# Boese0601/MagicDance

Hardware: NVIDIA H100
Metric: denoise-steps/sec @512x512 50-step DDIM (higher is better)
Workload: dtype f16

## Files before the change

include/magicdance_b200.h:

```cpp
#ifndef MAGICDANCE_B200_H_
#define MAGICDANCE_B200_H_

#include <stdint.h>

#ifdef __cplusplus
extern "C" {
#endif

#define MDB_OK 0
#define MDB_ERR_INVALID (-1)
#define MDB_ERR_CUDA (-2)
#define MDB_ERR_UNSUPPORTED (-3)

#define MDB_ABI_VERSION 2

typedef void* mdb_stream_t;

int mdb_abi_version(void);
const char* mdb_last_error(void);
int mdb_device_check(void);
int64_t mdb_launch_count(void);
int64_t mdb_abi_struct_bytes(int32_t which);

#define MDB_TUNE_GEMM_PAIR_MIN_TILES 1
#define MDB_TUNE_ATTN40_2Q_MIN_CTAS 3
#define MDB_TUNE_GEMM_BN80_BELOW 4
int mdb_set_tuning(int32_t key, int32_t value);
int32_t mdb_get_tuning(int32_t key);

#define MDB_EPI_NONE 0
#define MDB_EPI_GEGLU 1

typedef struct mdb_gemm_desc {
  const void* a;
  int64_t lda;
  const void* a2;
  int64_t lda2;
  int32_t k1;
  int32_t conv;
  int32_t nb, h, w, c;
  const void* b;
  int64_t ldb;
  void* d;
  int64_t ldd;
  const float* bias;
  int64_t bias_batch_stride;
  int32_t rows_per_batch;
  int32_t epilogue;
  const void* residual;
  int64_t ldr;
  int32_t m, n, k;
  int32_t splits;
  float* splitk_ws;
  const float* ln_u;
  float ln_eps;
} mdb_gemm_desc;

int mdb_gemm_f16(const mdb_gemm_desc* desc, mdb_stream_t stream);

#define MDB_DTYPE_F16 0
#define MDB_DTYPE_F32 1

typedef struct mdb_gemm_bwd_desc {
  mdb_gemm_desc fwd;
  const void* dd; int64_t lddd;
  void* da; int64_t ldda; int32_t da_dtype; int32_t da_accumulate;
  void* da2; int64_t ldda2; int32_t da2_dtype; int32_t da2_accumulate;
  void* db; int64_t lddb; int32_t db_dtype; int32_t db_accumulate;
  float* dbias; int32_t dbias_accumulate;
  int32_t splits;
  float* ws;
} mdb_gemm_bwd_desc;

int mdb_gemm_bwd_f16(const mdb_gemm_bwd_desc* desc, mdb_stream_t stream);
int64_t mdb_gemm_bwd_ws_floats(const mdb_gemm_bwd_desc* desc);

typedef struct mdb_attn_desc {
  const void* q; int64_t ldq;
  const void* k0; int64_t ldk0; const void* vt0; int64_t ldvt0; int32_t n0; int32_t kv0_batches; int32_t ldv0_batch;
  const void* k1; int64_t ldk1; const void* vt1; int64_t ldvt1; int32_t n1; int32_t kv1_batches; int32_t ldv1_batch;
  void* out; int64_t ldo;
  int32_t batch, heads, d, nq;
  int32_t bank_batches;
  float scale;
} mdb_attn_desc;

int mdb_attention_f16(const mdb_attn_desc* desc, mdb_stream_t stream);

int mdb_attention_lse_f16(const mdb_attn_desc* desc, float* lse, mdb_stream_t stream);

typedef struct mdb_attn_bwd_desc {
  mdb_attn_desc fwd;
  const void* dout; int64_t lddout;
  const float* lse;
  void* dq; int64_t lddq;
  void* dk0; int64_t lddk0; void* dvt0; int64_t lddvt0;
  void* dk1; int64_t lddk1; void* dvt1; int64_t lddvt1;
  float* ws;
} mdb_attn_bwd_desc;

int mdb_attention_bwd_f16(const mdb_attn_bwd_desc* desc, mdb_stream_t stream);
int64_t mdb_attention_bwd_ws_floats(int32_t batch, int32_t heads, int32_t nq);

int mdb_groupnorm_f16(const void* x1, int32_t c1, const void* x2, int32_t c2, const float* gamma, const float* beta,
                      void* y, float* ws, int32_t batch, int32_t hw, float eps, int32_t silu, int32_t mode,
                      mdb_stream_t stream);
int64_t mdb_groupnorm_ws_floats(int32_t c, int32_t batch, int32_t hw);

int mdb_layernorm_f16(const void* x, const float* gamma, const float* beta, void* y, int64_t rows, int32_t c,
                      float eps, mdb_stream_t stream);

typedef struct mdb_groupnorm_bwd_desc {
  const void* x1; const void* x2; int32_t c1; int32_t c2;
  const float* gamma; const float* beta;
  const void* dy;
  int32_t batch; int32_t hw; float eps; int32_t silu;
  void* dx1; int32_t dx1_dtype; int32_t dx1_accumulate;
  void* dx2; int32_t dx2_dtype; int32_t dx2_accumulate;
  float* dgamma; float* dbeta; int32_t dgamma_accumulate; int32_t dbeta_accumulate;
  float* ws;
} mdb_groupnorm_bwd_desc;

int mdb_groupnorm_bwd_f16(const mdb_groupnorm_bwd_desc* desc, mdb_stream_t stream);
int64_t mdb_groupnorm_bwd_ws_floats(const mdb_groupnorm_bwd_desc* desc);

typedef struct mdb_layernorm_bwd_desc {
  const void* x; const float* gamma; const void* dy;
  int64_t rows; int32_t c; float eps;
  void* dx; int32_t dx_dtype; int32_t dx_accumulate;
  float* dgamma; float* dbeta; int32_t dgamma_accumulate; int32_t dbeta_accumulate;
  float* ws;
} mdb_layernorm_bwd_desc;

int mdb_layernorm_bwd_f16(const mdb_layernorm_bwd_desc* desc, mdb_stream_t stream);
int64_t mdb_layernorm_bwd_ws_floats(const mdb_layernorm_bwd_desc* desc);

int mdb_geglu_f16(const void* h, int64_t ldh, void* out, int64_t ldo, int64_t m, int32_t n, mdb_stream_t stream);
int mdb_geglu_bwd_f16(const void* h, int64_t ldh, const void* dout, int64_t lddout, void* dh, int64_t lddh, int64_t m,
                      int32_t n, mdb_stream_t stream);

int mdb_conv3x3_direct_f16(const void* x, const void* wt, const float* bias, const void* residual, void* y,
                           int32_t batch, int32_t h, int32_t w, int32_t cin, int32_t cout, int32_t stride,
                           int32_t silu, mdb_stream_t stream);

typedef struct mdb_conv3x3_bwd_desc {
  const void* x; const void* wt; const void* wt_t; const float* bias; const void* dy;
  int32_t batch; int32_t h; int32_t w; int32_t cin; int32_t cout; int32_t stride; int32_t silu;
  void* dx;
  float* dw; int32_t dw_accumulate;
  float* dbias; int32_t dbias_accumulate;
  float* ws;
} mdb_conv3x3_bwd_desc;

int mdb_conv3x3_direct_bwd_f16(const mdb_conv3x3_bwd_desc* desc, mdb_stream_t stream);
int64_t mdb_conv3x3_direct_bwd_ws_floats(const mdb_conv3x3_bwd_desc* desc);

int mdb_im2col3x3_f16(const void* x, void* col, int32_t batch, int32_t h, int32_t w, int32_t c, int32_t stride,
                      mdb_stream_t stream);

int mdb_im2col3x3_br_f16(const void* x, void* col, int32_t batch, int32_t h, int32_t w, int32_t c, int32_t stride,
                         mdb_stream_t stream);

int mdb_upsample2x_f16(const void* x, void* y, int32_t batch, int32_t h, int32_t w, int32_t c, mdb_stream_t stream);
int mdb_upsample2x_bwd_f16(const void* dy, void* dx, int32_t dx_dtype, int32_t accumulate, int32_t batch, int32_t h,
                           int32_t w, int32_t c, mdb_stream_t stream);

int mdb_add_f16(const void* a, const void* b, void* y, int64_t n_per_batch, int32_t batch, int32_t b_batches,
                mdb_stream_t stream);

int mdb_timestep_embedding_f32(const int64_t* t, int32_t t_count, float* out, int32_t batch, int32_t dim,
                               mdb_stream_t stream);

int mdb_skinny_linear_f32(const float* x, const void* w, const float* bias, float* out, int32_t rows, int32_t n,
                          int32_t k, int32_t silu_in, int32_t silu_out, mdb_stream_t stream);

typedef struct mdb_skinny_linear_bwd_desc {
  const float* x; const void* w; const float* dy;
  int32_t rows; int32_t n; int32_t k; int32_t silu_in;
  float* dx; int32_t dx_accumulate;
  float* dw; int32_t dw_accumulate;
  float* dbias; int32_t dbias_accumulate;
// ... 21 lines not shown
```

magicdance_b200/_lib.py:

```python
from __future__ import annotations

import ctypes as C
import os

from . import build as _build

c_void_p, c_int32, c_int64, c_float = C.c_void_p, C.c_int32, C.c_int64, C.c_float


class GemmDesc(C.Structure):
    _fields_ = [
        ("a", c_void_p), ("lda", c_int64), ("a2", c_void_p), ("lda2", c_int64),
        ("k1", c_int32), ("conv", c_int32), ("nb", c_int32), ("h", c_int32), ("w", c_int32), ("c", c_int32),
        ("b", c_void_p), ("ldb", c_int64), ("d", c_void_p), ("ldd", c_int64),
        ("bias", c_void_p), ("bias_batch_stride", c_int64), ("rows_per_batch", c_int32), ("epilogue", c_int32),
        ("residual", c_void_p), ("ldr", c_int64),
        ("m", c_int32), ("n", c_int32), ("k", c_int32), ("splits", c_int32), ("splitk_ws", c_void_p),
        ("ln_u", c_void_p), ("ln_eps", c_float),
    ]


class AttnDesc(C.Structure):
    _fields_ = [
        ("q", c_void_p), ("ldq", c_int64),
        ("k0", c_void_p), ("ldk0", c_int64), ("vt0", c_void_p), ("ldvt0", c_int64),
        ("n0", c_int32), ("kv0_batches", c_int32), ("ldv0_batch", c_int32),
        ("k1", c_void_p), ("ldk1", c_int64), ("vt1", c_void_p), ("ldvt1", c_int64),
        ("n1", c_int32), ("kv1_batches", c_int32), ("ldv1_batch", c_int32),
        ("out", c_void_p), ("ldo", c_int64),
        ("batch", c_int32), ("heads", c_int32), ("d", c_int32), ("nq", c_int32), ("bank_batches", c_int32),
        ("scale", c_float),
    ]


class AttnBwdDesc(C.Structure):
    _fields_ = [
        ("fwd", AttnDesc),
        ("dout", c_void_p), ("lddout", c_int64),
        ("lse", c_void_p),
        ("dq", c_void_p), ("lddq", c_int64),
        ("dk0", c_void_p), ("lddk0", c_int64), ("dvt0", c_void_p), ("lddvt0", c_int64),
        ("dk1", c_void_p), ("lddk1", c_int64), ("dvt1", c_void_p), ("lddvt1", c_int64),
        ("ws", c_void_p),
    ]


class GemmBwdDesc(C.Structure):
    _fields_ = [
        ("fwd", GemmDesc),
        ("dd", c_void_p), ("lddd", c_int64),
        ("da", c_void_p), ("ldda", c_int64), ("da_dtype", c_int32), ("da_accumulate", c_int32),
        ("da2", c_void_p), ("ldda2", c_int64), ("da2_dtype", c_int32), ("da2_accumulate", c_int32),
        ("db", c_void_p), ("lddb", c_int64), ("db_dtype", c_int32), ("db_accumulate", c_int32),
        ("dbias", c_void_p), ("dbias_accumulate", c_int32),
        ("splits", c_int32),
        ("ws", c_void_p),
    ]


class GroupNormBwdDesc(C.Structure):
    _fields_ = [
        ("x1", c_void_p), ("x2", c_void_p), ("c1", c_int32), ("c2", c_int32),
        ("gamma", c_void_p), ("beta", c_void_p),
        ("dy", c_void_p),
        ("batch", c_int32), ("hw", c_int32), ("eps", c_float), ("silu", c_int32),
        ("dx1", c_void_p), ("dx1_dtype", c_int32), ("dx1_accumulate", c_int32),
        ("dx2", c_void_p), ("dx2_dtype", c_int32), ("dx2_accumulate", c_int32),
        ("dgamma", c_void_p), ("dbeta", c_void_p), ("dgamma_accumulate", c_int32), ("dbeta_accumulate", c_int32),
        ("ws", c_void_p),
    ]


class LayerNormBwdDesc(C.Structure):
    _fields_ = [
        ("x", c_void_p), ("gamma", c_void_p), ("dy", c_void_p),
        ("rows", c_int64), ("c", c_int32), ("eps", c_float),
        ("dx", c_void_p), ("dx_dtype", c_int32), ("dx_accumulate", c_int32),
        ("dgamma", c_void_p), ("dbeta", c_void_p), ("dgamma_accumulate", c_int32), ("dbeta_accumulate", c_int32),
        ("ws", c_void_p),
    ]


class Conv3x3BwdDesc(C.Structure):
    _fields_ = [
        ("x", c_void_p), ("wt", c_void_p), ("wt_t", c_void_p), ("bias", c_void_p), ("dy", c_void_p),
        ("batch", c_int32), ("h", c_int32), ("w", c_int32), ("cin", c_int32), ("cout", c_int32), ("stride", c_int32),
        ("silu", c_int32),
        ("dx", c_void_p),
        ("dw", c_void_p), ("dw_accumulate", c_int32),
        ("dbias", c_void_p), ("dbias_accumulate", c_int32),
        ("ws", c_void_p),
    ]


class SkinnyBwdDesc(C.Structure):
    _fields_ = [
        ("x", c_void_p), ("w", c_void_p), ("dy", c_void_p),
        ("rows", c_int32), ("n", c_int32), ("k", c_int32), ("silu_in", c_int32),
        ("dx", c_void_p), ("dx_accumulate", c_int32),
        ("dw", c_void_p), ("dw_accumulate", c_int32),
        ("dbias", c_void_p), ("dbias_accumulate", c_int32),
        ("ws", c_void_p),
    ]


SIGNATURES = {
    "mdb_abi_version": (c_int32, []),
    "mdb_last_error": (C.c_char_p, []),
    "mdb_device_check": (c_int32, []),
    "mdb_launch_count": (c_int64, []),
    "mdb_abi_struct_bytes": (c_int64, [c_int32]),
    "mdb_set_tuning": (c_int32, [c_int32, c_int32]),
    "mdb_get_tuning": (c_int32, [c_int32]),
    "mdb_gemm_f16": (c_int32, [C.POINTER(GemmDesc), c_void_p]),
    "mdb_gemm_bwd_f16": (c_int32, [C.POINTER(GemmBwdDesc), c_void_p]),
    "mdb_gemm_bwd_ws_floats": (c_int64, [C.POINTER(GemmBwdDesc)]),
    "mdb_attention_f16": (c_int32, [C.POINTER(AttnDesc), c_void_p]),
    "mdb_attention_lse_f16": (c_int32, [C.POINTER(AttnDesc), c_void_p, c_void_p]),
    "mdb_attention_bwd_f16": (c_int32, [C.POINTER(AttnBwdDesc), c_void_p]),
    "mdb_attention_bwd_ws_floats": (c_int64, [c_int32, c_int32, c_int32]),
    "mdb_groupnorm_f16": (c_int32, [c_void_p, c_int32, c_void_p, c_int32, c_void_p, c_void_p, c_void_p, c_void_p,
                                    c_int32, c_int32, c_float, c_int32, c_int32, c_void_p]),
    "mdb_groupnorm_ws_floats": (c_int64, [c_int32, c_int32, c_int32]),
    "mdb_layernorm_f16": (c_int32, [c_void_p, c_void_p, c_void_p, c_void_p, c_int64, c_int32, c_float, c_void_p]),
    "mdb_groupnorm_bwd_f16": (c_int32, [C.POINTER(GroupNormBwdDesc), c_void_p]),
    "mdb_groupnorm_bwd_ws_floats": (c_int64, [C.POINTER(GroupNormBwdDesc)]),
    "mdb_layernorm_bwd_f16": (c_int32, [C.POINTER(LayerNormBwdDesc), c_void_p]),
    "mdb_layernorm_bwd_ws_floats": (c_int64, [C.POINTER(LayerNormBwdDesc)]),
    "mdb_geglu_f16": (c_int32, [c_void_p, c_int64, c_void_p, c_int64, c_int64, c_int32, c_void_p]),
    "mdb_geglu_bwd_f16": (c_int32, [c_void_p, c_int64, c_void_p, c_int64, c_void_p, c_int64, c_int64, c_int32,
                                    c_void_p]),
    "mdb_conv3x3_direct_f16": (c_int32, [c_void_p, c_void_p, c_void_p, c_void_p, c_void_p, c_int32, c_int32, c_int32,
                                         c_int32, c_int32, c_int32, c_int32, c_void_p]),
    "mdb_conv3x3_direct_bwd_f16": (c_int32, [C.POINTER(Conv3x3BwdDesc), c_void_p]),
    "mdb_conv3x3_direct_bwd_ws_floats": (c_int64, [C.POINTER(Conv3x3BwdDesc)]),
    "mdb_im2col3x3_f16": (c_int32, [c_void_p, c_void_p, c_int32, c_int32, c_int32, c_int32, c_int32, c_void_p]),
    "mdb_im2col3x3_br_f16": (c_int32, [c_void_p, c_void_p, c_int32, c_int32, c_int32, c_int32, c_int32, c_void_p]),
    "mdb_upsample2x_f16": (c_int32, [c_void_p, c_void_p, c_int32, c_int32, c_int32, c_int32, c_void_p]),
    "mdb_upsample2x_bwd_f16": (c_int32, [c_void_p, c_void_p, c_int32, c_int32, c_int32, c_int32, c_int32, c_int32,
                                         c_void_p]),
    "mdb_add_f16": (c_int32, [c_void_p, c_void_p, c_void_p, c_int64, c_int32, c_int32, c_void_p]),
    "mdb_timestep_embedding_f32": (c_int32, [c_void_p, c_int32, c_void_p, c_int32, c_int32, c_void_p]),
    "mdb_skinny_linear_f32": (c_int32, [c_void_p, c_void_p, c_void_p, c_void_p, c_int32, c_int32, c_int32, c_int32,
                                        c_int32, c_void_p]),
    "mdb_skinny_linear_bwd_f32": (c_int32, [C.POINTER(SkinnyBwdDesc), c_void_p]),
    "mdb_skinny_linear_bwd_ws_floats": (c_int64, [C.POINTER(SkinnyBwdDesc)]),
    "mdb_nchw_f32_to_nhwc_f16": (c_int32, [c_void_p, c_void_p, c_int32, c_int32, c_int32, c_int32, c_int32, c_void_p]),
    "mdb_nhwc_f16_to_nchw_f32": (c_int32, [c_void_p, c_void_p, c_int32, c_int32, c_int32, c_int32, c_void_p]),
    "mdb_softmax_rows_f16": (c_int32, [c_void_p, c_int64, c_int32, c_int32, c_float, c_void_p]),
    "mdb_cfg_ddim_update_f32": (c_int32, [c_void_p, c_void_p, c_void_p, c_void_p, c_void_p, c_void_p, c_int64,
                                          c_void_p, c_int32, c_void_p]),
}

_lib = None
ABI_VERSION = 2
TUNE_GEMM_PAIR_MIN_TILES, TUNE_ATTN40_2Q_MIN_CTAS, TUNE_GEMM_BN80_BELOW = 1, 3, 4


def library_path() -> str:
    return os.environ.get("MAGICDANCE_B200_LIB", _build.LIB_PATH)


def load():
    global _lib
    if _lib is not None:
        return _lib
    path = library_path()
    if not os.path.isfile(path):
        raise RuntimeError(
            f"magicdance_b200: kernel library {path} is missing — run `python -m magicdance_b200.build` "
            "(there is no CPU/PyTorch fallback for the hot path)")
    if path == _build.LIB_PATH and os.path.isdir(_build.CSRC) and not _build.is_fresh():
        raise RuntimeError(f"magicdance_b200: {path} was not built from the sources in {_build.CSRC} "
                           "(stamp mismatch) — run `python -m magicdance_b200.build`")
    lib = C.CDLL(path)
    for name, (res, args) in SIGNATURES.items():
        fn = getattr(lib, name)
        fn.restype = res
        fn.argtypes = args
    if lib.mdb_abi_version() != ABI_VERSION:
        raise RuntimeError(f"magicdance_b200: ABI version mismatch ({lib.mdb_abi_version()} != {ABI_VERSION}); "
                           "rebuild the library")
    for which, mirror in ((0, GemmDesc), (1, AttnDesc), (2, AttnBwdDesc), (3, GemmBwdDesc), (4, GroupNormBwdDesc),
                          (5, LayerNormBwdDesc), (6, Conv3x3BwdDesc), (7, SkinnyBwdDesc)):
        if lib.mdb_abi_struct_bytes(which) != C.sizeof(mirror):
            raise RuntimeError(f"magicdance_b200: {mirror.__name__} mirrors {C.sizeof(mirror)} bytes, the library's "
                               f"struct has {lib.mdb_abi_struct_bytes(which)}: the binding and the library disagree")
    _lib = lib
    return lib


def check(rc: int, what: str):
    if rc != 0:
        msg = load().mdb_last_error().decode(errors="replace")
        raise RuntimeError(f"magicdance_b200.{what} failed (code {rc}): {msg}")
```

magicdance_b200/csrc/gemm.cu:

```cuda
#include <stdlib.h>

#include "common.cuh"

namespace mdb {

constexpr int kBM = 128;
constexpr int kBK = 64;

struct GemmKParams {
  CUtensorMap tmA;
  CUtensorMap tmA2;
  CUtensorMap tmB;
  __half* d;
  long long ldd;
  const float* bias;
  long long bias_batch_stride;
  const __half* residual;
  long long ldr;
  float* ws;
  int rows_per_batch;
  int m, n;
  int k_chunks;
  int k1_chunks;
  int chunks_per_split;
// ... 224 lines not shown
#pragma unroll
            for (int j = 0; j < 32; ++j)
              if (ch * 32 + j < BN) v[j] = lnst.y * fmaf(-lnst.x, s_lnu[ch * 32 + j], v[j]);
          }
          const int ncols = min(min(32, BN - ch * 32), p.n - col0);
          if (p.splits > 1) {
            if (row_ok) {
              float* wp = p.ws + (static_cast<long long>(split) * p.m + row) * p.n + col0;
#pragma unroll
              for (int j = 0; j < 32; j += 4) {
                if (j + 4 <= ncols && (p.n & 3) == 0) {
                  *reinterpret_cast<float4*>(wp + j) = make_float4(v[j], v[j + 1], v[j + 2], v[j + 3]);
                } else {
#pragma unroll
                  for (int e = 0; e < 4; ++e)
                    if (j + e < ncols) wp[j + e] = v[j + e];
                }
              }
            }
          } else if (row_ok) {
            const float* bias_chunk = nullptr;
            if (bias_in_smem) {
              bias_chunk = s_bias + ch * 32;
            } else if (p.bias != nullptr) {
              const long long brow = (p.bias_batch_stride != 0) ? (row / p.rows_per_batch) : 0;
              bias_chunk = p.bias + brow * p.bias_batch_stride + col0;
            }
            epi_store_chunk(p, row, col0, ncols, v, bias_chunk);
          }
        }
      }
    } else {
      const long long brow = (p.bias_batch_stride != 0) ? (row / p.rows_per_batch) : 0;
#pragma unroll 1
      for (int pr = half; pr < BN / 64; pr += 2) {
        const int col0 = n0 + pr * 64;
        if (col0 >= p.n) break;
        if (row_ok) {
          const float* bp = bias_in_smem ? (s_bias + pr * 64)
                                         : ((p.bias != nullptr) ? p.bias + brow * p.bias_batch_stride + col0 : nullptr);
          const float* rv = rrow + pr * 64;
          uint4* d4 = reinterpret_cast<uint4*>(p.d + row * p.ldd + (col0 >> 1));
#pragma unroll
          for (int q = 0; q < 4; ++q) {
            float o[8];
#pragma unroll
            for (int e = 0; e < 8; ++e) {
              const int j = q * 8 + e;
              float a = rv[j];
              float gt = rv[32 + j];
              if (bp != nullptr) {
                a += bp[j];
                gt += bp[32 + j];
              }
              o[e] = a * gelu_erf_f(gt);
            }
            uint4 o4;
            o4.x = pack_half2(o[0], o[1]);
            o4.y = pack_half2(o[2], o[3]);
            o4.z = pack_half2(o[4], o[5]);
            o4.w = pack_half2(o[6], o[7]);
            d4[q] = o4;
          }
        }
      }
    }
  }

  if constexpr (!GEGLU) {
    if (p.cluster_reduce) {
      const int S_ = p.splits;
      const int R = kBM / S_;
      const int groups = BN / 8;
      const uint32_t crank = cluster_ctarank();
      constexpr int kMaxItems = 4;
      uint4 rpre[kMaxItems];
      if (p.residual != nullptr) {
#pragma unroll
        for (int q = 0; q < kMaxItems; ++q) {
          const int item = threadIdx.x + q * kWsThreads;
          if (item < R * groups) {
            const int rl = item / groups, cgp = item - rl * groups;
            const long long row = static_cast<long long>(m0) + static_cast<int>(crank) * R + rl;
            const int col0 = n0 + cgp * 8;
            if (row < p.m && col0 + 8 <= p.n) rpre[q] = *reinterpret_cast<const uint4*>(p.residual + row * p.ldr + col0);
          }
        }
      }
      cluster_sync_all();
      const uint32_t red_base = smem_u32(smem);
#pragma unroll 1
      for (int it_ = 0; it_ * kWsThreads < R * groups; ++it_) {
        const int item = threadIdx.x + it_ * kWsThreads;
        if (item >= R * groups) break;
        const int rl = item / groups, cgp = item - rl * groups;
        const int rt = static_cast<int>(crank) * R + rl;
        const long long row = static_cast<long long>(m0) + rt;
        const int col0 = n0 + cgp * 8;
        if (row >= p.m || col0 >= p.n) continue;
        const uint32_t off = red_base + static_cast<uint32_t>((rt * kRedLd + cgp * 8) * 4);
        float o[8];
#pragma unroll
        for (int e = 0; e < 8; ++e) o[e] = 0.f;
        for (int pr = 0; pr < S_; ++pr) {
          const uint32_t ra = dsmem_map(off, static_cast<uint32_t>(pr));
          const float4 a = dsmem_ld_f4(ra), b = dsmem_ld_f4(ra + 16);
          o[0] += a.x; o[1] += a.y; o[2] += a.z; o[3] += a.w;
          o[4] += b.x; o[5] += b.y; o[6] += b.z; o[7] += b.w;
        }
        const int ncols = min(8, p.n - col0);
        const long long brow = (p.bias_batch_stride != 0) ? (row / p.rows_per_batch) : 0;
        if (p.bias != nullptr) {
          const float* bp = p.bias + brow * p.bias_batch_stride + col0;
          for (int e = 0; e < ncols; ++e) o[e] += bp[e];
        }
        if (ncols == 8) {
          if (p.residual != nullptr) {
            uint4 r4 = make_uint4(0, 0, 0, 0);
            if (it_ < kMaxItems) {
#pragma unroll
              for (int q = 0; q < kMaxItems; ++q)
                if (q == it_) r4 = rpre[q];
            } else {
              r4 = *reinterpret_cast<const uint4*>(p.residual + row * p.ldr + col0);
            }
            const __half2* h2 = reinterpret_cast<const __half2*>(&r4);
#pragma unroll
            for (int e = 0; e < 4; ++e) {
              const float2 f = __half22float2(h2[e]);
              o[2 * e] += f.x;
              o[2 * e + 1] += f.y;
            }
          }
          uint4 o4;
          o4.x = pack_half2(o[0], o[1]);
          o4.y = pack_half2(o[2], o[3]);
          o4.z = pack_half2(o[4], o[5]);
          o4.w = pack_half2(o[6], o[7]);
          *reinterpret_cast<uint4*>(p.d + row * p.ldd + col0) = o4;
        } else {
          for (int e = 0; e < ncols; ++e) {
            float x = o[e];
            if (p.residual != nullptr) x += __half2float(p.residual[row * p.ldr + col0 + e]);
            p.d[row * p.ldd + col0 + e] = __float2half_rn(x);
          }
        }
      }
      cluster_sync_all();
    }
  }

}

__global__ void splitk_finalize_kernel(GemmKParams p) {
  pdl_launch_dependents();
  pdl_wait();
  const long long slab = static_cast<long long>(p.m) * p.n;
  if ((p.n & 3) == 0) {
    const long long total4 = slab >> 2;
    for (long long i = static_cast<long long>(blockIdx.x) * blockDim.x + threadIdx.x; i < total4;
         i += static_cast<long long>(gridDim.x) * blockDim.x) {
      const long long e = i << 2;
      const long long row = e / p.n;
      const int col = static_cast<int>(e - row * p.n);
      float4 a = *reinterpret_cast<const float4*>(p.ws + e);
      for (int s = 1; s < p.splits; ++s) {
        const float4 b = *reinterpret_cast<const float4*>(p.ws + s * slab + e);
        a.x += b.x; a.y += b.y; a.z += b.z; a.w += b.w;
      }
      if (p.bias != nullptr) {
        const long long brow = (p.bias_batch_stride != 0) ? (row / p.rows_per_batch) : 0;
        const float* bp = p.bias + brow * p.bias_batch_stride + col;
        a.x += bp[0]; a.y += bp[1]; a.z += bp[2]; a.w += bp[3];
      }
      if (p.residual != nullptr) {
        const __half2* rp = reinterpret_cast<const __half2*>(p.residual + row * p.ldr + col);
        const float2 r0 = __half22float2(rp[0]), r1 = __half22float2(rp[1]);
        a.x += r0.x; a.y += r0.y; a.z += r1.x; a.w += r1.y;
      }
      uint2 o;
      o.x = pack_half2(a.x, a.y);
      o.y = pack_half2(a.z, a.w);
      *reinterpret_cast<uint2*>(p.d + row * p.ldd + col) = o;
    }
    return;
  }
  for (long long i = static_cast<long long>(blockIdx.x) * blockDim.x + threadIdx.x; i < slab;
       i += static_cast<long long>(gridDim.x) * blockDim.x) {
    const long long row = i / p.n;
    const int col = static_cast<int>(i - row * p.n);
    float v = 0.f;
    for (int s = 0; s < p.splits; ++s) v += p.ws[s * slab + i];
    if (p.bias != nullptr) {
      const long long brow = (p.bias_batch_stride != 0) ? (row / p.rows_per_batch) : 0;
      v += p.bias[brow * p.bias_batch_stride + col];
    }
    if (p.residual != nullptr) v += __half2float(p.residual[row * p.ldr + col]);
    p.d[row * p.ldd + col] = __float2half_rn(v);
  }
}

int pixel_box(int ho, int wo, int cs, int rows, bool fwd, uint32_t box[4]) {
  const int hw = ho * wo;
  if (fwd ? wo > rows : wo >= rows) {
    if (wo % rows || (fwd && cs != 1)) return kBoxWideRows;
    box[1] = cs * rows; box[2] = 1; box[3] = 1;
  } else if (hw >= rows) {
    if (rows % wo || hw % rows) return kBoxRowsPerTile;
    box[1] = cs * wo; box[2] = cs * (rows / wo); box[3] = 1;
  } else {
    if (rows % hw) return kBoxImagesPerTile;
    box[1] = cs * wo; box[2] = cs * ho; box[3] = rows / hw;
  }
  box[0] = 64;
  return box[1] <= 256 && box[2] <= 256 ? kBoxOk : kBoxTooLarge;
}

static int g_pair_min_tiles = 128;
static int g_bn80_below = 100;
constexpr int kLongKChunks = 64;

template <int BN, bool GEGLU, int STAGES>
static int launch_gemm(const GemmKParams& kp, dim3 grid, cudaStream_t st) {
  const unsigned cluster_z = kp.cluster_reduce ? static_cast<unsigned>(kp.splits) : 1u;
  constexpr auto kern = gemm_tc_kernel<BN, GEGLU, STAGES>;
  constexpr int kSmem = GemmSmem<BN, STAGES>::kTotal;
  static_assert(kSmem <= 227 * 1024, "shared memory budget");
  if (int rc = set_max_dyn_smem<kern>(kSmem)) return rc;
  MDB_CHECK_CUDA(launch_pdl_cluster(kern, grid, dim3(kWsThreads), kSmem, st, cluster_z, kp));
  count_launch();
  return MDB_OK;
}

int get_gemm_tuning(int key) { return key == MDB_TUNE_GEMM_PAIR_MIN_TILES ? g_pair_min_tiles : g_bn80_below; }
void set_gemm_tuning(int key, int value) {
  if (key == MDB_TUNE_GEMM_PAIR_MIN_TILES) g_pair_min_tiles = value;
  else g_bn80_below = value;
}

}

using namespace mdb;

extern "C" int mdb_gemm_f16(const mdb_gemm_desc* g, mdb_stream_t stream) {
  MDB_REQUIRE(g != nullptr, "mdb_gemm_f16: null descriptor");
  MDB_REQUIRE(g->m > 0 && g->n > 0 && g->k > 0, "mdb_gemm_f16: bad shape m=%d n=%d k=%d", g->m, g->n, g->k);
  MDB_REQUIRE(g->k % kBK == 0, "mdb_gemm_f16: K=%d must be a multiple of 64", g->k);
  MDB_REQUIRE(g->a && g->b && g->d, "mdb_gemm_f16: null operand");
  cudaStream_t st = static_cast<cudaStream_t>(stream);
  const bool geglu = g->epilogue == MDB_EPI_GEGLU;
  GemmKParams kp;
  memset(&kp, 0, sizeof(kp));
  kp.d = static_cast<__half*>(g->d);
  kp.ldd = g->ldd;
  kp.bias = g->bias;
  kp.bias_batch_stride = g->bias_batch_stride;
  kp.rows_per_batch = g->rows_per_batch > 0 ? g->rows_per_batch : 1;
  kp.residual = static_cast<const __half*>(g->residual);
  kp.ldr = g->ldr;
  kp.m = g->m;
  kp.n = g->n;
  kp.k_chunks = g->k / kBK;
  kp.conv = g->conv;
  MDB_REQUIRE(g->ldd % 8 == 0 && (reinterpret_cast<uintptr_t>(g->d) & 15) == 0,
              "mdb_gemm_f16: D must be 16B aligned with ldd %% 8 == 0 (ldd=%lld)", (long long)g->ldd);
  if (g->bias) {
    MDB_REQUIRE((reinterpret_cast<uintptr_t>(g->bias) & 15) == 0 && g->bias_batch_stride % 4 == 0,
                "mdb_gemm_f16: bias must be 16B aligned with bias_batch_stride %% 4 == 0");
  }
  if (g->residual) {
    MDB_REQUIRE(g->ldr % 8 == 0 && (reinterpret_cast<uintptr_t>(g->residual) & 15) == 0,
                "mdb_gemm_f16: residual must be 16B aligned with ldr %% 8 == 0");
    MDB_REQUIRE(!geglu, "mdb_gemm_f16: residual is not supported with the GEGLU epilogue");
  }

  if (g->ln_u != nullptr) {
    MDB_REQUIRE(!geglu, "mdb_gemm_f16: LayerNorm fusion is not available with the GEGLU epilogue (N / 128 CTAs per row "
                        "block would each recompute the row statistics: measured slower than the LayerNorm kernel)");
    MDB_REQUIRE(!g->conv && g->a2 == nullptr && (reinterpret_cast<uintptr_t>(g->ln_u) & 15) == 0,
                "mdb_gemm_f16: LayerNorm fusion needs a plain single-source A whose K is the normalised width");
    kp.ln_u = g->ln_u;
    kp.ln_eps = g->ln_eps;
  }
  int rc;
  if (g->conv) {
    MDB_REQUIRE(g->a2 == nullptr, "mdb_gemm_f16: conv mode takes a single source");
    MDB_REQUIRE(g->c % kBK == 0 && g->k == 9 * g->c, "mdb_gemm_f16: conv needs c %% 64 == 0 and k == 9c (c=%d k=%d)",
                g->c, g->k);
    const int cs = g->conv == 2 ? 2 : 1;
    const int ho = (g->h - 1) / cs + 1, wo = (g->w - 1) / cs + 1;
    MDB_REQUIRE(g->m == g->nb * ho * wo, "mdb_gemm_f16: conv m != nb*ho*wo");
    const int hw = ho * wo;
    uint32_t box[4];
    const int why = pixel_box(ho, wo, cs, kBM, true, box);
    MDB_REQUIRE(why != kBoxWideRows, "mdb_gemm_f16: conv rows wider than 128 pixels need 128 | w and stride 1 (w=%d)", g->w);
    MDB_REQUIRE(why != kBoxRowsPerTile, "mdb_gemm_f16: conv tile needs w | 128 and 128 | h*w (output h=%d w=%d)", ho, wo);
    MDB_REQUIRE(why != kBoxImagesPerTile, "mdb_gemm_f16: conv tile needs h*w | 128 (output h=%d w=%d)", ho, wo);
    MDB_REQUIRE(why != kBoxTooLarge, "mdb_gemm_f16: conv TMA box too large");
    rc = tmap_nhwc(&kp.tmA, g->a, g->c, g->w, g->h, g->nb, g->c, box, cs);
    if (rc) return rc;
    kp.chunks_per_tap = g->c / kBK;
    kp.w = wo;
    kp.hw = hw;
    kp.cs = cs;
    kp.k1_chunks = kp.k_chunks;
  } else {
    const int k1 = g->a2 ? g->k1 : g->k;
    MDB_REQUIRE(k1 % kBK == 0 && k1 > 0 && k1 <= g->k, "mdb_gemm_f16: k1=%d must be a multiple of 64 within K", k1);
    rc = tmap_rows(&kp.tmA, g->a, k1, g->m, g->lda, kBK, kBM);
    if (rc) return rc;
    if (g->a2) {
      rc = tmap_rows(&kp.tmA2, g->a2, g->k - k1, g->m, g->lda2, kBK, kBM);
      if (rc) return rc;
    }
    kp.k1_chunks = k1 / kBK;
  }

  const int m_tiles = (g->m + kBM - 1) / kBM;
  bool pair = g->splits <= 1 && m_tiles >= 2 && g->n % 8 == 0 && g->ln_u == nullptr;
  int bn = 0;
  if (pair) {
    if (geglu) bn = (g->n % 256 == 0) ? 256 : 0;
    else if (g->n % 256 == 0) bn = 256;
    else if (g->n % 160 == 0) bn = 160;
    else bn = 128;
    const long long eq = (long long)m_tiles * ((g->n + bn - 1) / (bn ? bn : 1));
    if (bn == 0 || eq < (long long)g_pair_min_tiles || eq * kp.k_chunks < 16ll * g_pair_min_tiles) pair = false;
  }
  if (pair) {
  } else if (geglu) {
    MDB_REQUIRE(g->n % 128 == 0, "mdb_gemm_f16: GEGLU needs N %% 128 == 0 (N=%d)", g->n);
    bn = 128;
  } else if (g->n % 160 == 0) {
    const long long tiles160 = (long long)m_tiles * (g->n / 160) * (g->splits > 1 ? g->splits : 1);
    const bool wide_split = g->splits == 0 && kp.k_chunks >= kLongKChunks && tiles160 * 2 <= kNumSms;
    bn = (tiles160 < g_bn80_below && !wide_split) ? 80 : 160;
  } else {
    bn = 128;
  }
  rc = tmap_rows(&kp.tmB, g->b, g->k, g->n, g->ldb, kBK, bn);
  if (rc) return rc;

  int splits = g->splits > 1 ? g->splits : 1;
  if (g->ln_u != nullptr) splits = 1;
  if (g->splits == 0 && !geglu && !pair && g->ln_u == nullptr) {
    const long long tiles = (long long)m_tiles * ((g->n + bn - 1) / bn);
    if (tiles < 100)
      for (int c = 8; c >= 2; c >>= 1)
        if (tiles * c <= kNumSms && kp.k_chunks / c >= 16) {
          splits = c;
          break;
        }
  }
  if (splits > kp.k_chunks) splits = kp.k_chunks;
  if (geglu || pair) splits = 1;
  kp.chunks_per_split = (kp.k_chunks + splits - 1) / splits;
  splits = (kp.k_chunks + kp.chunks_per_split - 1) / kp.chunks_per_split;
  kp.splits = splits;
  kp.ws = g->splitk_ws;
  kp.cluster_reduce = (!geglu && (splits == 2 || splits == 4 || splits == 8)) ? 1 : 0;
  if (splits > 1 && !kp.cluster_reduce) {
    MDB_REQUIRE(g->splitk_ws != nullptr, "mdb_gemm_f16: splits > 1 needs splitk_ws");
  }

  dim3 grid(m_tiles, (g->n + bn - 1) / bn, splits);
  const bool deep = (long long)grid.x * grid.y * grid.z <= kNumSms && kp.chunks_per_split >= 12;
  if (pair) {
    if (bn == 256) rc = geglu ? launch_gemm<256, true, 4>(kp, grid, st) : launch_gemm<256, false, 4>(kp, grid, st);
    else if (bn == 160) rc = launch_gemm<160, false, 6>(kp, grid, st);
    else rc = launch_gemm<128, false, 6>(kp, grid, st);
    return rc;
  }
  if (geglu) rc = launch_gemm<128, true, 3>(kp, grid, st);
  else if (bn == 160) rc = deep ? launch_gemm<160, false, 6>(kp, grid, st) : launch_gemm<160, false, 3>(kp, grid, st);
  else if (bn == 80) rc = deep ? launch_gemm<80, false, 8>(kp, grid, st) : launch_gemm<80, false, 3>(kp, grid, st);
  else rc = deep ? launch_gemm<128, false, 6>(kp, grid, st) : launch_gemm<128, false, 3>(kp, grid, st);
  if (rc) return rc;
  if (splits > 1 && !kp.cluster_reduce) {
    const long long total = ((long long)g->m * g->n + 3) / 4;
    int blocks = (int)((total + 255) / 256);
    if (blocks > kNumSms * 8) blocks = kNumSms * 8;
    MDB_CHECK_CUDA(launch_pdl(splitk_finalize_kernel, dim3(blocks), dim3(256), 0, st, kp));
    count_launch();
  }
  return MDB_OK;
}
```

magicdance_b200/ops.py:

```python
from __future__ import annotations

import ctypes as C
import os

import torch

from . import _lib

EPI_NONE, EPI_GEGLU = 0, 1
SKINNY_MAX_ROWS = 16
_GEMM_DEBUG = os.environ.get("MDB_GEMM_DEBUG", "0") == "1"
TRACE = None


class tuning:
    _KEYS = {"pair_min_tiles": _lib.TUNE_GEMM_PAIR_MIN_TILES,
             "attn40_2q_min_ctas": _lib.TUNE_ATTN40_2Q_MIN_CTAS, "bn80_below": _lib.TUNE_GEMM_BN80_BELOW}

    def __init__(self, **kw):
        self.want = {self._KEYS[k]: int(v) for k, v in kw.items() if v is not None}

    def __enter__(self):
        lib = _lib.load()
        self.old = {k: int(lib.mdb_get_tuning(k)) for k in self.want}
        for k, v in self.want.items():
            _lib.check(lib.mdb_set_tuning(k, v), "set_tuning")
        return self

    def __exit__(self, *a):
        lib = _lib.load()
        for k, v in self.old.items():
            lib.mdb_set_tuning(k, v)


def _stream() -> int:
    return torch.cuda.current_stream().cuda_stream


def _ptr(t):
    return None if t is None else t.data_ptr()


def _chk(t: torch.Tensor, dtype, name):
    if not t.is_cuda:
        raise RuntimeError(f"magicdance_b200: {name} must be a CUDA tensor (no CPU fallback exists for the hot path)")
    if t.dtype != dtype:
        raise RuntimeError(f"magicdance_b200: {name} must be {dtype}, got {t.dtype}")


def require_cuda(device):
    if torch.device(device).type != "cuda":
        raise RuntimeError("magicdance_b200: the networks run only on an sm_90 CUDA device — move the model to "
                           "the GPU first (there is no CPU/PyTorch fallback for the hot path)")


def ensure_device():
    lib = _lib.load()
    if not torch.cuda.is_available():
        raise RuntimeError("magicdance_b200: no CUDA device visible; the hot path has no CPU fallback")
    _lib.check(lib.mdb_device_check(), "device_check")
    return lib


def launch_count() -> int:
    return int(_lib.load().mdb_launch_count())


_ws_cache = {}


_ws_tag = 0


class workspace_lane:

    def __init__(self, tag):
        self.tag = tag

    def __enter__(self):
        global _ws_tag
        self.prev, _ws_tag = _ws_tag, self.tag

    def __exit__(self, *a):
        global _ws_tag
        _ws_tag = self.prev


def current_lane():
    return _ws_tag


_ws_retired = []


def _workspace(key, numel, dtype, device, zero=False):
    k = (key, device, _ws_tag)
    t = _ws_cache.get(k)
    if t is None or t.numel() < numel or t.dtype != dtype:
        if t is not None:
            _ws_retired.append(t)
            numel = max(numel, 2 * t.numel())
        alloc = torch.zeros if zero else torch.empty
        t = alloc(max(numel, 1), dtype=dtype, device=device)
        _ws_cache[k] = t
    return t


def _gemm_m(a, conv, conv_stride, m):
    if conv is not None:
        nb, h, wd, _ = conv
        return nb * ((h - 1) // conv_stride + 1) * ((wd - 1) // conv_stride + 1)
    return a.shape[0] if m is None else m


def _fill_fwd_desc(g, a, w, a2, conv, conv_stride, m):
    n, k = w.shape
    if conv is not None:
        nb, h, wd, c = conv
        assert conv_stride in (1, 2) and a.is_contiguous() and a.numel() == nb * h * wd * c
        g.conv, g.nb, g.h, g.w, g.c = conv_stride, nb, h, wd, c
        g.a, g.lda, g.k1 = a.data_ptr(), c, k
    else:
        assert a.dim() == 2 and a.stride(1) == 1
        g.a, g.lda, g.k1 = a.data_ptr(), a.stride(0), a.shape[1]
        if a2 is not None:
            _chk(a2, torch.float16, "a2")
            assert a2.dim() == 2 and a2.stride(1) == 1 and a2.shape[0] == a.shape[0]
            g.a2, g.lda2 = a2.data_ptr(), a2.stride(0)
            assert a.shape[1] + a2.shape[1] == k
        else:
            assert a.shape[1] == k, (a.shape, w.shape)
    m = _gemm_m(a, conv, conv_stride, m)
    g.m, g.n, g.k = m, n, k
    return m, g.k1


def gemm(a, w, *, out=None, bias=None, bias_batch_stride=0, rows_per_batch=0, residual=None, epilogue=EPI_NONE,
         a2=None, conv=None, conv_stride=1, splits=0, m=None, ln_u=None, ln_eps=1e-5):
    lib = _lib.load()
    _chk(a, torch.float16, "a")
    _chk(w, torch.float16, "w")
    g = _lib.GemmDesc()
    n, k = w.shape
    m, _ = _fill_fwd_desc(g, a, w, a2, conv, conv_stride, m)
    n_out = n // 2 if epilogue == EPI_GEGLU else n
    if out is None:
        out = torch.empty((m, n_out), dtype=torch.float16, device=a.device)
    _chk(out, torch.float16, "out")
    assert out.dim() == 2 and out.stride(1) == 1 and out.shape[0] >= m and out.shape[1] == n_out, (out.shape, m, n_out)
    assert w.stride(1) == 1
    g.b, g.ldb = w.data_ptr(), w.stride(0)
    g.d, g.ldd = out.data_ptr(), out.stride(0)
    if bias is not None:
        _chk(bias, torch.float32, "bias")
        g.bias, g.bias_batch_stride, g.rows_per_batch = bias.data_ptr(), bias_batch_stride, rows_per_batch
    if residual is not None:
        _chk(residual, torch.float16, "residual")
        assert residual.dim() == 2 and residual.stride(1) == 1
        g.residual, g.ldr = residual.data_ptr(), residual.stride(0)
    g.epilogue = epilogue
    if ln_u is not None:
        _chk(ln_u, torch.float32, "ln_u")
        assert conv is None and a2 is None and ln_u.numel() == n and ln_u.is_contiguous()
        g.ln_u, g.ln_eps = ln_u.data_ptr(), float(ln_eps)
        splits = 1
    if TRACE is not None:
        TRACE.append((m, n, k, (tuple(conv) + (conv_stride,)) if conv is not None else None, epilogue, splits,
                      a2.shape[1] if a2 is not None else 0))
    if splits > 1:
        ws = _workspace("splitk", splits * m * n, torch.float32, a.device)
        g.splits, g.splitk_ws = splits, ws.data_ptr()
    else:
        g.splits = splits
    if _GEMM_DEBUG:
        import sys
        print(f"gemm m={m} n={n} k={k} conv={conv} epi={epilogue} splits={g.splits} a2={a2 is not None} lda={g.lda} "
              f"ldd={g.ldd} bias={bias is not None} bbs={g.bias_batch_stride} res={residual is not None}",
              file=sys.stderr, flush=True)
    _lib.check(lib.mdb_gemm_f16(C.byref(g), _stream()), "gemm_f16")
    if _GEMM_DEBUG:
        torch.cuda.synchronize()
    return out


_DTYPES = {torch.float16: 0, torch.float32: 1}
# ... 754 lines not shown
```

Baseline: 89.57.

## Add persistent warp-specialized GEMM kernel with per-warp swizzled smem epilogue

Adds a persistent GEMM kernel that launches at most one CTA per SM and loops over output tiles. The TMA producer warp keeps streaming the next tile's K-chunks while consumer warpgroups run the epilogue of the current tile. The epilogue stages accumulators through a per-warp swizzled shared-memory buffer so each lane writes coalesced 16-byte stores, with bias and residual added on the way. This path is on by default for non-split, non-GEGLU, non-LN GEMMs on the pair/deep paths and can be switched off from Python. The cost is extra shared memory and less tile-level parallelism when there are few tiles.

```diff
diff --git a/include/magicdance_b200.h b/include/magicdance_b200.h
--- a/include/magicdance_b200.h
+++ b/include/magicdance_b200.h
@@ -27,6 +27,7 @@
 #define MDB_TUNE_GEMM_BN80_BELOW 4
 int mdb_set_tuning(int32_t key, int32_t value);
 int32_t mdb_get_tuning(int32_t key);
+int32_t mdb_set_gemm_persistent(int32_t on);
 
 #define MDB_EPI_NONE 0
 #define MDB_EPI_GEGLU 1
diff --git a/magicdance_b200/_lib.py b/magicdance_b200/_lib.py
--- a/magicdance_b200/_lib.py
+++ b/magicdance_b200/_lib.py
@@ -112,6 +112,7 @@
     "mdb_abi_struct_bytes": (c_int64, [c_int32]),
     "mdb_set_tuning": (c_int32, [c_int32, c_int32]),
     "mdb_get_tuning": (c_int32, [c_int32]),
+    "mdb_set_gemm_persistent": (c_int32, [c_int32]),
     "mdb_gemm_f16": (c_int32, [C.POINTER(GemmDesc), c_void_p]),
     "mdb_gemm_bwd_f16": (c_int32, [C.POINTER(GemmBwdDesc), c_void_p]),
     "mdb_gemm_bwd_ws_floats": (c_int64, [C.POINTER(GemmBwdDesc)]),
diff --git a/magicdance_b200/csrc/gemm.cu b/magicdance_b200/csrc/gemm.cu
--- a/magicdance_b200/csrc/gemm.cu
+++ b/magicdance_b200/csrc/gemm.cu
@@ -400,6 +400,171 @@
 
 }
 
+template <int BN, int STAGES>
+struct GemmPersistSmem {
+  static constexpr int kRing = GemmSmem<BN, STAGES>::kStageBytes * STAGES;
+  static constexpr int kEC = (kRing + 1024 + (kConsumers / 32) * 16 * 32 * 4 <= 225 * 1024) ? 32 : 16;
+  static constexpr int kWarpFloats = 16 * kEC;
+  static constexpr int kTotal = kRing + (kConsumers / 32) * kWarpFloats * 4 + 1024;
+};
+
+template <int EC>
+__device__ __forceinline__ int epi_idx(int r, int c) {
+  constexpr int kGranules = EC / 4;
+  const int sw = (r / (32 / EC)) & (kGranules - 1);
+  return r * EC + (((c >> 2) ^ sw) << 2) + (c & 3);
+}
+
+template <int BN, int EC, int C0, int W>
+__device__ __forceinline__ void persist_epi_chunk(const GemmKParams& p, const float (&acc)[BN / 2], float* stage,
+                                                  int row0, int n0, int lane) {
+  constexpr int kJ0 = C0 / 2;
+  const int fr = lane >> 2, fc = 2 * (lane & 3);
+  __syncwarp();
+#pragma unroll
+  for (int j = kJ0; j < kJ0 + W / 2; j += 2) {
+    const int r = fr + 8 * ((j >> 1) & 1);
+    const int c = 8 * (j >> 2) + fc - C0;
+    *reinterpret_cast<float2*>(stage + epi_idx<EC>(r, c)) = make_float2(acc[j], acc[j + 1]);
+  }
+  __syncwarp();
+  constexpr int kLanesPerRow = W / 8;
+  constexpr int kRowsPerPass = 32 / kLanesPerRow;
+  const int t = lane % kLanesPerRow;
+  const int col0 = n0 + C0 + 8 * t;
+  if (col0 >= p.n) return;
+#pragma unroll
+  for (int pass = 0; pass < 16 / kRowsPerPass; ++pass) {
+    const int r = pass * kRowsPerPass + lane / kLanesPerRow;
+    const int row = row0 + r;
+    if (row >= p.m) break;
+    const float4 lo = *reinterpret_cast<const float4*>(stage + epi_idx<EC>(r, 8 * t));
+    const float4 hi = *reinterpret_cast<const float4*>(stage + epi_idx<EC>(r, 8 * t + 4));
+    float o[8] = {lo.x, lo.y, lo.z, lo.w, hi.x, hi.y, hi.z, hi.w};
+    if (p.bias != nullptr) {
+      const long long brow = (p.bias_batch_stride != 0) ? (row / p.rows_per_batch) : 0;
+      const float* bp = p.bias + brow * p.bias_batch_stride + col0;
+      const float4 b0 = *reinterpret_cast<const float4*>(bp);
+      const float4 b1 = *reinterpret_cast<const float4*>(bp + 4);
+      o[0] += b0.x; o[1] += b0.y; o[2] += b0.z; o[3] += b0.w;
+      o[4] += b1.x; o[5] += b1.y; o[6] += b1.z; o[7] += b1.w;
+    }
+    if (p.residual != nullptr) {
+      const uint4 r4 = *reinterpret_cast<const uint4*>(p.residual + static_cast<long long>(row) * p.ldr + col0);
+      const __half2* h2 = reinterpret_cast<const __half2*>(&r4);
+#pragma unroll
+      for (int e = 0; e < 4; ++e) {
+        const float2 f = __half22float2(h2[e]);
+        o[2 * e] += f.x;
+        o[2 * e + 1] += f.y;
+      }
+    }
+    uint4 o4;
+    o4.x = pack_half2(o[0], o[1]);
+    o4.y = pack_half2(o[2], o[3]);
+    o4.z = pack_half2(o[4], o[5]);
+    o4.w = pack_half2(o[6], o[7]);
+    *reinterpret_cast<uint4*>(p.d + static_cast<long long>(row) * p.ldd + col0) = o4;
+  }
+}
+
+template <int BN, int EC, int C0>
+__device__ __forceinline__ void persist_epilogue(const GemmKParams& p, const float (&acc)[BN / 2], float* stage,
+                                                 int row0, int n0, int lane) {
+  if constexpr (C0 < BN) {
+    constexpr int W = BN - C0 < EC ? BN - C0 : EC;
+    if (n0 + C0 < p.n) persist_epi_chunk<BN, EC, C0, W>(p, acc, stage, row0, n0, lane);
+    persist_epilogue<BN, EC, C0 + W>(p, acc, stage, row0, n0, lane);
+  }
+}
+
+template <int BN, int kStages>
+__global__ void __launch_bounds__(kWsThreads, 1) gemm_tc_persistent_kernel(const __grid_constant__ GemmKParams p) {
+  using S = GemmSmem<BN, kStages>;
+  using P = GemmPersistSmem<BN, kStages>;
+  extern __shared__ uint8_t smem_raw[];
+  __shared__ __align__(8) uint64_t full_bar[kStages];
+  __shared__ __align__(8) uint64_t empty_bar[kStages];
+
+  uint8_t* smem = align1024(smem_raw);
+  const int warp = threadIdx.x >> 5;
+  const int lane = threadIdx.x & 31;
+  const int m_tiles = (p.m + kBM - 1) / kBM;
+  const int tiles = m_tiles * ((p.n + BN - 1) / BN);
+  const int n_iter = p.k_chunks;
+
+  pdl_launch_dependents();
+  if (warp == kProducerWarp && lane == 0) {
+    tma_prefetch_desc(&p.tmA);
+    tma_prefetch_desc(&p.tmB);
+    ring_init<kStages>(full_bar, empty_bar, 1);
+    fence_barrier_init();
+  }
+  __syncthreads();
+  pdl_wait();
+
+  if (warp == kProducerWarp) {
+    if (lane == 0) {
+      int g = 0;
+      for (int tile = blockIdx.x; tile < tiles; tile += gridDim.x) {
+        const int m0 = (tile % m_tiles) * kBM;
+        const int n0 = (tile / m_tiles) * BN;
+        int b0 = 0, y0 = 0, x0 = 0;
+        if (p.conv) {
+          b0 = m0 / p.hw;
+          y0 = (p.hw >= kBM) ? (m0 % p.hw) / p.w : 0;
+          x0 = (p.hw >= kBM) ? (m0 % p.hw) % p.w : 0;
+        }
+        for (int kc = 0; kc < n_iter; ++kc, ++g) {
+          const int s = ring_acquire<kStages>(empty_bar, g);
+          uint8_t* sa = smem + s * S::kStageBytes;
+          uint8_t* sb = sa + S::kABytes;
+          mbar_expect_tx(&full_bar[s], S::kStageBytes);
+          if (p.conv) {
+            const int tap = kc / p.chunks_per_tap;
+            const int cc = kc - tap * p.chunks_per_tap;
+            const int kh = tap / 3, kw = tap - kh * 3;
+            tma_load_4d(sa, &p.tmA, &full_bar[s], cc * kBK, p.cs * x0 + kw - 1, p.cs * y0 + kh - 1, b0);
+          } else if (kc < p.k1_chunks) {
+            tma_load_2d(sa, &p.tmA, &full_bar[s], kc * kBK, m0);
+          } else {
+            tma_load_2d(sa, &p.tmA2, &full_bar[s], (kc - p.k1_chunks) * kBK, m0);
+          }
+          tma_load_2d(sb, &p.tmB, &full_bar[s], kc * kBK, n0);
+        }
+      }
+    }
+  } else {
+    const int wg = warp >> 2;
+    float* stage = reinterpret_cast<float*>(smem + P::kRing) + warp * P::kWarpFloats;
+    int g = 0;
+    for (int tile = blockIdx.x; tile < tiles; tile += gridDim.x) {
+      const int m0 = (tile % m_tiles) * kBM;
+      const int n0 = (tile / m_tiles) * BN;
+      float acc[BN / 2];
+#pragma unroll
+      for (int i = 0; i < BN / 2; ++i) acc[i] = 0.f;
+      for (int it = 0; it < n_iter; ++it, ++g) {
+        const int s = ring_wait_full<kStages>(full_bar, g);
+        const uint32_t a_addr = smem_u32(smem + s * S::kStageBytes);
+        const uint64_t da = wgmma_desc_k_sw128(a_addr + wg * (64 * 128));
+        const uint64_t db = wgmma_desc_k_sw128(a_addr + S::kABytes);
+        wgmma_fence();
+#pragma unroll
+        for (int k = 0; k < kBK / 16; ++k) wgmma_ss<BN>(acc, da + 2 * k, db + 2 * k, 1u);
+        wgmma_commit();
+        wgmma_wait<1>();
+        wgmma_fence_regs(acc);
+        if (it > 0) mbar_arrive(&empty_bar[(g - 1) % kStages]);
+      }
+      wgmma_wait<0>();
+      wgmma_fence_regs(acc);
+      mbar_arrive(&empty_bar[(g - 1) % kStages]);
+      persist_epilogue<BN, P::kEC, 0>(p, acc, stage, m0 + warp * 16, n0, lane);
+    }
+  }
+}
+
 __global__ void splitk_finalize_kernel(GemmKParams p) {
   pdl_launch_dependents();
   pdl_wait();
@@ -466,6 +631,7 @@
 
 static int g_pair_min_tiles = 128;
 static int g_bn80_below = 100;
+static int g_persistent = 1;
 constexpr int kLongKChunks = 64;
 
 template <int BN, bool GEGLU, int STAGES>
@@ -480,6 +646,19 @@
   return MDB_OK;
 }
 
+template <int BN, int STAGES>
+static int launch_gemm_persistent(const GemmKParams& kp, dim3 grid, cudaStream_t st) {
+  constexpr auto kern = gemm_tc_persistent_kernel<BN, STAGES>;
+  constexpr int kSmem = GemmPersistSmem<BN, STAGES>::kTotal;
+  static_assert(kSmem <= 227 * 1024, "shared memory budget");
+  if (int rc = set_max_dyn_smem<kern>(kSmem)) return rc;
+  const long long tiles = (long long)grid.x * grid.y;
+  MDB_CHECK_CUDA(launch_pdl(kern, dim3(static_cast<unsigned>(tiles < kNumSms ? tiles : kNumSms)), dim3(kWsThreads),
+                            kSmem, st, kp));
+  count_launch();
+  return MDB_OK;
+}
+
 int get_gemm_tuning(int key) { return key == MDB_TUNE_GEMM_PAIR_MIN_TILES ? g_pair_min_tiles : g_bn80_below; }
 void set_gemm_tuning(int key, int value) {
   if (key == MDB_TUNE_GEMM_PAIR_MIN_TILES) g_pair_min_tiles = value;
@@ -489,6 +668,12 @@
 }
 
 using namespace mdb;
+
+extern "C" int32_t mdb_set_gemm_persistent(int32_t on) {
+  const int32_t prev = g_persistent;
+  g_persistent = on != 0;
+  return prev;
+}
 
 extern "C" int mdb_gemm_f16(const mdb_gemm_desc* g, mdb_stream_t stream) {
   MDB_REQUIRE(g != nullptr, "mdb_gemm_f16: null descriptor");
@@ -613,6 +798,12 @@
 
   dim3 grid(m_tiles, (g->n + bn - 1) / bn, splits);
   const bool deep = (long long)grid.x * grid.y * grid.z <= kNumSms && kp.chunks_per_split >= 12;
+  if (g_persistent && splits == 1 && g->ln_u == nullptr && g->n % 8 == 0 && !geglu && (pair || deep)) {
+    if (bn == 256) return launch_gemm_persistent<256, 4>(kp, grid, st);
+    if (bn == 160) return launch_gemm_persistent<160, 6>(kp, grid, st);
+    if (bn == 80) return launch_gemm_persistent<80, 8>(kp, grid, st);
+    return launch_gemm_persistent<128, 6>(kp, grid, st);
+  }
   if (pair) {
     if (bn == 256) rc = geglu ? launch_gemm<256, true, 4>(kp, grid, st) : launch_gemm<256, false, 4>(kp, grid, st);
     else if (bn == 160) rc = launch_gemm<160, false, 6>(kp, grid, st);
diff --git a/magicdance_b200/ops.py b/magicdance_b200/ops.py
--- a/magicdance_b200/ops.py
+++ b/magicdance_b200/ops.py
@@ -16,21 +16,29 @@
 class tuning:
     _KEYS = {"pair_min_tiles": _lib.TUNE_GEMM_PAIR_MIN_TILES,
              "attn40_2q_min_ctas": _lib.TUNE_ATTN40_2Q_MIN_CTAS, "bn80_below": _lib.TUNE_GEMM_BN80_BELOW}
+    _SWITCHES = ("gemm_persistent",)
 
     def __init__(self, **kw):
-        self.want = {self._KEYS[k]: int(v) for k, v in kw.items() if v is not None}
+        unknown = set(kw) - set(self._KEYS) - set(self._SWITCHES)
+        if unknown:
+            raise KeyError(f"ops.tuning: unknown keys {sorted(unknown)}")
+        self.want = {self._KEYS[k]: int(v) for k, v in kw.items() if v is not None and k in self._KEYS}
+        self.persistent = kw.get("gemm_persistent")
 
     def __enter__(self):
         lib = _lib.load()
         self.old = {k: int(lib.mdb_get_tuning(k)) for k in self.want}
         for k, v in self.want.items():
             _lib.check(lib.mdb_set_tuning(k, v), "set_tuning")
+        self.old_persistent = None if self.persistent is None else int(lib.mdb_set_gemm_persistent(int(self.persistent)))
         return self
 
     def __exit__(self, *a):
         lib = _lib.load()
         for k, v in self.old.items():
             lib.mdb_set_tuning(k, v)
+        if self.old_persistent is not None:
+            lib.mdb_set_gemm_persistent(self.old_persistent)
 
 
 def _stream() -> int:
```

After: 90.26, median of 6. About the same (+0.8%).
